# Neela08/cloud-security-pytorch-sagemaker-distributed-workshop

Hardware: AMD Instinct MI355X
Metric: images/sec (whole node) ResNet-50 DDP (higher is better)
Workload: dtype bf16; 1 GPU; model=resnet50, global_batch=256, per_gpu_batch=256, image_size=224, parallelism=dp1, optimizer=SGD(momentum=0.9, wd=1e-4), fp32 master weights, bf16 compute, backend=none, launcher=none, device=cuda, comm_forced_at_world1=False, buckets=5, grad_comm=fp32, wgrad_stream=True, hip_graph=False, gpu_max_hw_queues=8

## Files before the change

### csrc/kernels/gemm_conv.hip

```cpp
#include "common.h"
#include "epilogue.h"
#include <algorithm>
#include <array>
#include <climits>
#include <cstdio>
#include <vector>
#include <mutex>
#include <cstdlib>

constexpr int kNtBlocksPerCu = 4, kNt64BlocksPerCu = 4;
constexpr int kTnBlocksPerCu = 3, kTnConvBlocksPerCu = 3;
constexpr int kNtEpiEU = 4;

namespace {

struct ConvGeom {
  int H, W, Cs;
  int P, Q;
  int R, S, stride, pad;
  FastDiv fPQ, fQ, fS, fCpt;
  int Pc[4], Qc[4];
  FastDiv fPQc[4], fQc[4];
};

// ... 599 lines not shown
        float f[8];
        unpack8(v, f);
        if (a.epi == 5) {
          float c0[8];
          unpack8(cv[sl][u], c0);
#pragma unroll
          for (int q = 0; q < 8; ++q) f[q] += c0[q];
        }
        if constexpr (MASKC) {
          float xv[8];
          unpack8(xq[sl][u], xv);
#pragma unroll
          for (int q = 0; q < 8; ++q) {
            const float t = mthr[MASKC ? q : 0];
            const bool keep = ((mgt >> q) & 1u) ? xv[q] > t : xv[q] < t;
            f[q] = keep ? f[q] : 0.f;
          }
        } else if (a.bn_relu && a.mbits) {
#pragma unroll
          for (int q = 0; q < 8; ++q) f[q] = ((yq[sl][u].x >> q) & 1u) ? f[q] : 0.f;
        } else if (a.bn_relu) {
          float yv[8];
          unpack8(yq[sl][u], yv);
#pragma unroll
          for (int q = 0; q < 8; ++q) f[q] = yv[q] > 0.f ? f[q] : 0.f;
        }
        o = pack8(f);
        if (a.stats) {
          float xv[8];
          unpack8(xq[sl][u], xv);
#pragma unroll
          for (int q = 0; q < 8; ++q) { s1[q] += f[q]; s2[q] += f[q] * (xv[q] - mu[q]); }
        }
      } else {
        if (a.epi) o = epilogue_op_v(a.epi, v, a.aux + off, yq[sl][u]);
        if (a.stats) {
          float f[8];
          unpack8(v, f);
#pragma unroll
          for (int q = 0; q < 8; ++q) { s1[q] += f[q]; s2[q] += f[q] * f[q]; }
        }
      }
      *(uint4*)((bf16_t*)a.C + off) = o;
    }
  };
#pragma unroll
  for (int g = 0; g < NG; ++g) {
    load_grp(g, 0);
    proc_grp(g, 0);
  }
  if (a.stats) {
#pragma unroll
    for (int o = CPR; o < 64; o <<= 1) {
#pragma unroll
      for (int q = 0; q < 8; ++q) {
        s1[q] += __shfl_xor(s1[q], o, 64);
        s2[q] += __shfl_xor(s2[q], o, 64);
      }
    }
    if (lane < CPR) {
#pragma unroll
      for (int q = 0; q < 8; ++q) {
        Sred[(wid * 2 + 0) * BN + cc * 8 + q] = s1[q];
        Sred[(wid * 2 + 1) * BN + cc * 8 + q] = s2[q];
      }
    }
    __syncthreads();
    const int prow = cy * a.tiles_m + tm;
    for (int c = tid; c < 2 * BN; c += 256) {
      const int which = c / BN, col = c - which * BN;
      float t = 0.f;
#pragma unroll
      for (int w = 0; w < 4; ++w) t += Sred[(w * 2 + which) * BN + col];
      if (n0 + col < a.N) a.stats[((size_t)prow * 2 + which) * a.N + n0 + col] = t;
    }
  }
}

template <int UNITS>
__device__ __forceinline__ int tr_swz(int k) {
  return (4 * (k & 3) + 16 * ((k >> 3) & 1)) & (UNITS - 1);
}

template <int BM, int BN, int STAGES, int MODE = 1, bool CS = false, bool NOL = false, bool CSB = false>
__global__ __launch_bounds__(256, STAGES == 1 ? (MODE == 1 && !CS ? kTnConvBlocksPerCu : kTnBlocksPerCu) : 2)
void tn_kernel(TNArgs a) {
  static_assert(!CSB || (STAGES == 1 && !CS && !NOL), "folded BN backward: the plain one-stage variant");
  static_assert(!NOL || (MODE == 1 && STAGES == 1 && !CS), "normalize-on-load: conv weight gradients");
  constexpr int WM = BM / 2, WN = BN / 2;
  constexpr int MI = WM / 16, NJ = WN / 16;
  constexpr int AU = BM / 4, BU = BN / 4;
  constexpr int ACPR = BM / 8, BCPR = BN / 8;
  constexpr int A_CH = BK * ACPR / 256, B_CH = BK * BCPR / 256;
  constexpr int A_RSTEP = 256 / ACPR, B_RSTEP = 256 / BCPR;
  constexpr int A_RPI = 64 / ACPR, B_RPI = 64 / BCPR;
  __shared__ __attribute__((aligned(16))) uint2 smem[STAGES * BK * (AU + BU)];
  uint2* As = smem;
  uint2* Bs = smem + STAGES * BK * AU;

  const int nbn = (a.N + BN - 1) / BN;
  const int tiles = ((a.M + BM - 1) / BM) * nbn;
  const int nsplit = gridDim.x / tiles;
  const int w = xcd_remap(blockIdx.x, gridDim.x);
  const int split = w / tiles, tile = w - split * tiles;
  const int m0 = (tile / nbn) * BM, n0 = (tile % nbn) * BN;
  const int kbeg = split * a.k_per_split;
  const int kend = min(a.K, kbeg + a.k_per_split);
  if (kbeg >= kend) return;

  const int tid = threadIdx.x, lane = tid & 63, wid = tid >> 6;
  const int wm = wid >> 1, wn = wid & 1;
  const int a_cc = tid % ACPR, a_r = tid / ACPR;
  const int b_cc = tid % BCPR, b_r = tid / BCPR;
  const int a_lc = a_cc ^ (tr_swz<AU>(a_r) >> 1);
  const int b_lc = b_cc ^ (tr_swz<BU>(b_r) >> 1);

  int tap_r = 0, tap_s = 0, c0 = 0;
  if constexpr (MODE == 1) {
    const int ncol = n0 + b_lc * 8;
    const int tap = ncol / a.g.Cs;
    c0 = ncol - tap * a.g.Cs;
    tap_r = tap / a.g.S;
    tap_s = tap - tap_r * a.g.S;
  }
  const int H = a.g.H, W = a.g.W, P = a.g.P, Q = a.g.Q, Cs = a.g.Cs;
  const int st = a.g.stride, pad = a.g.pad;
  float nsc[NOL ? 8 : 1], nsh[NOL ? 8 : 1];
  if constexpr (NOL) {
    const bool live = n0 + b_lc * 8 < a.N;
#pragma unroll
    for (int q = 0; q < 8; ++q) {
      nsc[q] = live ? a.nol_scale[c0 + q] : 0.f;
      nsh[q] = live ? a.nol_shift[c0 + q] : 0.f;
    }
  }

  int b_img[B_CH], b_p[B_CH], b_q[B_CH];
#pragma unroll
  for (int i = 0; i < B_CH; ++i) {
    const uint32_t k = (uint32_t)min(kbeg + b_r + B_RSTEP * i, a.K - 1);
    if constexpr (MODE == 1) {
      const uint32_t img = fdiv(k, a.g.fPQ);
      const uint32_t rem = k - img * a.g.fPQ.d;
      const uint32_t p = fdiv(rem, a.g.fQ);
      b_img[i] = (int)img; b_p[i] = (int)p; b_q[i] = (int)(rem - p * a.g.fQ.d);
    } else {
      b_img[i] = b_p[i] = b_q[i] = 0;
    }
  }
  const int dq = BK % Q, dp = (BK / Q) % P, dimg = BK / (P * Q);

  const bool a_second = CSB && a.msplit && m0 >= a.msplit;
  const __amdgpu_buffer_rsrc_t rsA = __builtin_amdgcn_make_buffer_rsrc(
      (void*)(a_second ? a.A2 : a.A), (short)0, a_second ? a.a2_bytes : a.a_bytes, 0x00020000);
  const __amdgpu_buffer_rsrc_t rsB = __builtin_amdgcn_make_buffer_rsrc((void*)a.B, (short)0, a.b_bytes, 0x00020000);
  constexpr uint32_t OOB = 0xFFFFFFF0u;
  const int a_m = m0 + a_lc * 8;
  const int a_mo = a_second ? a_m - a.msplit : a_m;
  const int b_n = n0 + b_lc * 8;

  uint32_t b_okm = 0;
  auto issue_loads = [&](int k0, int buf) {
    b_okm = 0;
#pragma unroll
    for (int i = 0; i < A_CH; ++i) {
      const int k = k0 + a_r + A_RSTEP * i;
      const bool ok = k < kend && a_m < a.M;
      const uint32_t vo = ok ? (uint32_t)(k * (a_second ? a.lda2 : a.lda) + a_mo) * 2u : OOB;
      __builtin_amdgcn_raw_ptr_buffer_load_lds(
          rsA, LDS_PTR(void, &As[(buf * BK + A_RSTEP * i + wid * A_RPI) * AU]), 16, vo, 0, 0, 0);
    }
#pragma unroll
    for (int i = 0; i < B_CH; ++i) {
      const int k = k0 + b_r + B_RSTEP * i;
      uint32_t vo = OOB;
      if constexpr (MODE == 0) {
        if (k < kend && b_n < a.N) vo = (uint32_t)(k * a.ldb + b_n) * 2u;
      } else {
        const int ih = b_p[i] * st - pad + tap_r, iw = b_q[i] * st - pad + tap_s;
        if (k < kend && (unsigned)ih < (unsigned)H && (unsigned)iw < (unsigned)W)
          vo = (b_n < a.N) ? (uint32_t)((((b_img[i] * H + ih) * W + iw) * Cs) + c0) * 2u : OOB;
        b_okm |= (vo != OOB ? 1u : 0u) << i;
        int q = b_q[i] + dq, p = b_p[i] + dp, img = b_img[i] + dimg;
        if (q >= Q) { q -= Q; ++p; }
        if (p >= P) { p -= P; ++img; }
        b_q[i] = q; b_p[i] = p; b_img[i] = img;
      }
      __builtin_amdgcn_raw_ptr_buffer_load_lds(
          rsB, LDS_PTR(void, &Bs[(buf * BK + B_RSTEP * i + wid * B_RPI) * BU]), 16, vo, 0, 0, 0);
    }
  };

  f32x4 acc[MI][NJ];
#pragma unroll
  for (int i = 0; i < MI; ++i)
#pragma unroll
    for (int j = 0; j < NJ; ++j) acc[i][j] = f32x4{0.f, 0.f, 0.f, 0.f};

  const int g = lane >> 4, li = lane & 15, q4 = li >> 2, p4 = li & 3;
  const bool do_cs = CS && (tile % nbn) == 0 && wn == 0;
  f32x4 acc_cs[CS ? MI : 1];
#pragma unroll
  for (int i = 0; i < (CS ? MI : 1); ++i) acc_cs[i] = f32x4{0.f, 0.f, 0.f, 0.f};
  short ones_s __attribute__((ext_vector_type(8))) = {0x3F80, 0x3F80, 0x3F80, 0x3F80,
                                                      0x3F80, 0x3F80, 0x3F80, 0x3F80};
  const bf16x8 ones = __builtin_bit_cast(bf16x8, ones_s);
  const bool do_csb = CSB && tile / nbn == 0 && wm == 0;
  f32x4 acc_sb[CSB ? NJ : 1];
#pragma unroll
  for (int j = 0; j < (CSB ? NJ : 1); ++j) acc_sb[j] = f32x4{0.f, 0.f, 0.f, 0.f};
  auto compute = [&](int cur) {
#pragma unroll
    for (int kk = 0; kk < 2; ++kk) {
      bf16x8 af[MI], bfr[NJ];
      const int k1 = kk * 32 + 8 * g + q4;
      const int k2 = k1 + 4;
#pragma unroll
      for (int i = 0; i < MI; ++i) {
        const int u = (wm * WM + 16 * i) / 4 + p4;
        short4v lo = __builtin_amdgcn_ds_read_tr16_b64_v4i16(LDS_PTR(short4v, &As[(cur * BK + k1) * AU + (u ^ tr_swz<AU>(k1))]));
        short4v hi = __builtin_amdgcn_ds_read_tr16_b64_v4i16(LDS_PTR(short4v, &As[(cur * BK + k2) * AU + (u ^ tr_swz<AU>(k2))]));
        short v8 __attribute__((ext_vector_type(8))) = {lo[0], lo[1], lo[2], lo[3], hi[0], hi[1], hi[2], hi[3]};
        af[i] = __builtin_bit_cast(bf16x8, v8);
      }
#pragma unroll
      for (int j = 0; j < NJ; ++j) {
        const int u = (wn * WN + 16 * j) / 4 + p4;
        short4v lo = __builtin_amdgcn_ds_read_tr16_b64_v4i16(LDS_PTR(short4v, &Bs[(cur * BK + k1) * BU + (u ^ tr_swz<BU>(k1))]));
        short4v hi = __builtin_amdgcn_ds_read_tr16_b64_v4i16(LDS_PTR(short4v, &Bs[(cur * BK + k2) * BU + (u ^ tr_swz<BU>(k2))]));
        short v8 __attribute__((ext_vector_type(8))) = {lo[0], lo[1], lo[2], lo[3], hi[0], hi[1], hi[2], hi[3]};
        bfr[j] = __builtin_bit_cast(bf16x8, v8);
      }
#pragma unroll
      for (int i = 0; i < MI; ++i)
#pragma unroll
        for (int j = 0; j < NJ; ++j)
          acc[i][j] = __builtin_amdgcn_mfma_f32_16x16x32_bf16(af[i], bfr[j], acc[i][j], 0, 0, 0);
      if constexpr (CS) {
        if (do_cs)
#pragma unroll
        for (int i = 0; i < MI; ++i) acc_cs[i] = __builtin_amdgcn_mfma_f32_16x16x32_bf16(af[i], ones, acc_cs[i], 0, 0, 0);
      }
      if constexpr (CSB) {
        if (do_csb)
#pragma unroll
        for (int j = 0; j < NJ; ++j) acc_sb[j] = __builtin_amdgcn_mfma_f32_16x16x32_bf16(ones, bfr[j], acc_sb[j], 0, 0, 0);
      }
    }
  };

  const int nk = (kend - kbeg + BK - 1) / BK;
  if constexpr (STAGES == 1) {
    for (int kt = 0; kt < nk; ++kt) {
      issue_loads(kbeg + kt * BK, 0);
      asm volatile("s_waitcnt vmcnt(0)" ::: "memory");
      if constexpr (NOL) {
#pragma unroll
        for (int i = 0; i < B_CH; ++i) {
          if (!((b_okm >> i) & 1u)) continue;
          uint4* p = (uint4*)&Bs[(B_RSTEP * i + wid * B_RPI) * BU + 2 * lane];
          float f[8];
          unpack8(*p, f);
#pragma unroll
          for (int q = 0; q < 8; ++q) f[q] = fmaxf(fmaf(f[q], nsc[q], nsh[q]), 0.f);
          *p = pack8(f);
        }
      }
      __syncthreads();
      compute(0);
      __syncthreads();
    }
  } else {
    issue_loads(kbeg, 0);
    asm volatile("s_waitcnt vmcnt(0)" ::: "memory");
    __syncthreads();
    for (int kt = 0; kt < nk; ++kt) {
      const int cur = kt & 1;
      if (kt + 1 < nk) issue_loads(kbeg + (kt + 1) * BK, cur ^ 1);
      compute(cur);
      asm volatile("s_waitcnt vmcnt(0)" ::: "memory");
      __syncthreads();
    }
  }

  if constexpr (CS) if (do_cs && li == 0) {
#pragma unroll
    for (int i = 0; i < MI; ++i)
#pragma unroll
      for (int r = 0; r < 4; ++r) {
        const int m = m0 + wm * WM + 16 * i + 4 * g + r;
        if (m < a.M) atomicAdd(a.colsum + m, acc_cs[i][r]);
      }
  }

  if constexpr (CSB) if (do_csb && g == 0) {
#pragma unroll
    for (int j = 0; j < NJ; ++j) {
      const int n = n0 + wn * WN + 16 * j + li;
      if (n < a.N) a.bsum[(size_t)split * a.N + n] = acc_sb[j][0];
    }
  }

  const bool single = (nsplit == 1);
  if (!single && a.ws) {
    if (STAGES == 1 && a.cnt) {
      constexpr int FR = BM * BN / 4;
      constexpr int SC1 = 16;
      const __amdgpu_buffer_rsrc_t rsw = __builtin_amdgcn_make_buffer_rsrc(
          a.ws + (size_t)tile * nsplit * FR * 4, (short)0, nsplit * FR * 16, 0x00020000);
#pragma unroll
      for (int i = 0; i < MI; ++i)
#pragma unroll
        for (int j = 0; j < NJ; ++j)
          __builtin_amdgcn_raw_buffer_store_b128(
              acc[i][j], rsw, (uint32_t)((split * FR + ((i * NJ + j) * 4 + wid) * 64 + lane) * 16), 0, SC1);
      asm volatile("s_waitcnt vmcnt(0)" ::: "memory");
      __syncthreads();
      __shared__ int last_flag;
      if (tid == 0) last_flag = atomicAdd(a.cnt + tile, 1) == nsplit - 1;
      __syncthreads();
      if (!last_flag) return;
#pragma unroll
      for (int i = 0; i < MI; ++i)
#pragma unroll
        for (int j = 0; j < NJ; ++j) acc[i][j] = f32x4{0.f, 0.f, 0.f, 0.f};
      constexpr int IU = MI >= 2 ? MI / 2 : 1;
      for (int z = 0; z < nsplit; ++z) {
#pragma unroll
        for (int i0 = 0; i0 < MI; i0 += IU) {
          f32x4 r[IU][NJ];
#pragma unroll
          for (int i = 0; i < IU; ++i)
#pragma unroll
            for (int j = 0; j < NJ; ++j)
              r[i][j] = __builtin_amdgcn_raw_buffer_load_b128(
                  rsw, (uint32_t)((z * FR + (((i0 + i) * NJ + j) * 4 + wid) * 64 + lane) * 16), 0, SC1);
#pragma unroll
          for (int i = 0; i < IU; ++i)
#pragma unroll
            for (int j = 0; j < NJ; ++j) acc[i0 + i][j] += r[i][j];
        }
      }
      if (tid == 0) a.cnt[tile] = 0;
#pragma unroll
      for (int i = 0; i < MI; ++i) {
#pragma unroll
        for (int j = 0; j < NJ; ++j) {
          const int n = n0 + wn * WN + 16 * j + li;
          if (n >= a.N) continue;
          float c[4];
#pragma unroll
          for (int r = 0; r < 4; ++r) c[r] = a.C[(size_t)min(m0 + wm * WM + 16 * i + 4 * g + r, a.M - 1) * a.ldc + n];
#pragma unroll
          for (int r = 0; r < 4; ++r) {
            const int m = m0 + wm * WM + 16 * i + 4 * g + r;
            if (m < a.M) a.C[(size_t)m * a.ldc + n] = c[r] + acc[i][j][r];
          }
        }
      }
      return;
    }
    f32x4* slab = (f32x4*)a.ws + ((size_t)tile * nsplit + split) * (BM * BN / 4);
#pragma unroll
    for (int i = 0; i < MI; ++i)
#pragma unroll
      for (int j = 0; j < NJ; ++j) {
        f32x4* q = slab + ((i * NJ + j) * 4 + wid) * 64 + lane;
        *q = acc[i][j];
      }
  } else {
#pragma unroll
    for (int i = 0; i < MI; ++i) {
#pragma unroll
      for (int j = 0; j < NJ; ++j) {
        const int n = n0 + wn * WN + 16 * j + li;
        if (n >= a.N) continue;
#pragma unroll
        for (int r = 0; r < 4; ++r) {
          const int m = m0 + wm * WM + 16 * i + 4 * g + r;
          if (m >= a.M) continue;
          float* dst = a.C + (size_t)m * a.ldc + n;
          if (single) *dst += acc[i][j][r];
          else atomicAdd(dst, acc[i][j][r]);
        }
      }
    }
  }
}
// ... 393 lines not shown
                       int stats, int blocks, int splits) {
  if (g_trace_gemm < 0) {
    const char* e = std::getenv("MI355X_DP_TRACE_GEMM");
    g_trace_gemm = (e && e[0] == '1') ? 1 : 0;
  }
  if (!g_trace_gemm) return;
  static std::vector<std::array<int, 12>> seen;
  const std::array<int, 12> key{(int)(intptr_t)what, mode, M, N, K, Cs, R, stride, epi, stats, blocks, splits};
  for (auto& k : seen)
    if (k == key) return;
  seen.push_back(key);
  fprintf(stderr, "[gemm] %s mode=%d M=%d N=%d K=%d Cs=%d R=%d s=%d epi=%d stats=%d blocks=%d splits=%d\n", what,
          mode, M, N, K, Cs, R, stride, epi, stats, blocks, splits);
}

hipError_t dispatch_nt(NTArgs& a, hipStream_t st, const ConvRoute& r) {
  const ConvGeom& g = a.g;
  if (r.k == ConvKernel::NtHalo) {
    a.halo_rp = r.halo_rp;
    a.halo_pb = cdiv(g.P, r.halo_rp);
    a.fPB = make_fastdiv((uint32_t)a.halo_pb);
    a.fHW2 = make_fastdiv((uint32_t)(g.Q + 2));
    trace_gemm(r.bn == 64 ? "nt128x64-halo" : "nt128x128-halo", a.mode, a.M, a.N, a.K, g.Cs, g.R, g.stride, a.epi,
               a.stats != nullptr, (a.M / (g.P * g.Q)) * a.halo_pb, 1);
  } else {
    trace_gemm(r.bm == 64 ? "nt64x64" : (r.bn == 64 ? "nt128x64" : "nt128x128"), a.mode, a.M, a.N, a.K, g.Cs, g.R,
               g.stride, a.epi, a.stats != nullptr, cdiv(a.M, r.bm) * cdiv(a.N, r.bn), a.mode == 3 ? a.ncls : 1);
  }
  if (r.bm == 64) return launch_nt<64, 64>(a, st);
  return r.bn == 64 ? launch_nt<128, 64>(a, st) : launch_nt<128, 128>(a, st);
}
hipError_t dispatch_nt(NTArgs& a, hipStream_t st) { return dispatch_nt(a, st, nt_route(a.M, a.N)); }

struct SplitkWs { float* p = nullptr; size_t n = 0; };
static SplitkWs g_splitk_ws[16][3];
static hipStream_t g_wgrad_stream[16];
static hipStream_t g_aux_stream[16];
static std::mutex g_splitk_mu;
static float* splitk_workspace(size_t floats, hipStream_t st) {
  int dev = 0;
  hipGetDevice(&dev);
  std::lock_guard<std::mutex> lk(g_splitk_mu);
  const int slot = st == nullptr ? 0 : st == g_wgrad_stream[dev & 15] ? 1 : st == g_aux_stream[dev & 15] ? 2 : 0;
  SplitkWs& w = g_splitk_ws[dev & 15][slot];
  if (w.n < floats) {
    if (mi_stream_capturing(st)) {
      mi_ws_capture_warn("split-K slab");
      return nullptr;
    }
    const size_t n = std::max(floats, (size_t)16 << 20);
    float* p = nullptr;
    if (hipMalloc(&p, n * sizeof(float)) != hipSuccess) return nullptr;
    mi_ws_retire(w.p);
    w.p = p;
    w.n = n;
  }
  return w.p;
}
static int* g_splitk_cnt[16][3];
static int* splitk_counters(hipStream_t st) {
  int dev = 0;
  hipGetDevice(&dev);
  std::lock_guard<std::mutex> lk(g_splitk_mu);
  const int slot = st == nullptr ? 0 : st == g_wgrad_stream[dev & 15] ? 1 : st == g_aux_stream[dev & 15] ? 2 : 0;
  int*& p = g_splitk_cnt[dev & 15][slot];
  if (!p) {
    if (hipMalloc(&p, sizeof(int) * SPLITK_COUNTERS) != hipSuccess) { p = nullptr; return nullptr; }
    if (hipMemset(p, 0, sizeof(int) * SPLITK_COUNTERS) != hipSuccess) return nullptr;
  }
  return p;
}
extern "C" float* mi_partials_workspace(size_t floats, hipStream_t st) { return splitk_workspace(floats, st); }
MI_API int mi_splitk_ws_reserve(size_t floats, hipStream_t st) { return splitk_workspace(floats, st) ? 0 : 1; }
static int g_tn_slabs = -1;
static bool tn_slabs_on() {
  if (g_tn_slabs < 0) {
    const char* e = std::getenv("MI355X_DP_TN_SLABS");
    g_tn_slabs = (e && e[0] == '0') ? 0 : 1;
  }
  return g_tn_slabs != 0;
}

static int g_tn_stages = -1;
static int tn_stages() {
  if (g_tn_stages < 0) {
    const char* e = std::getenv("MI355X_DP_TN_STAGES");
    g_tn_stages = (e && e[0] == '2') ? 2 : 1;
  }
  return g_tn_stages;
}

template <int BM, int BN>
hipError_t launch_tn(TNArgs& a, hipStream_t st, int target_blocks) {
  int tiles = cdiv(a.M, BM) * cdiv(a.N, BN);
  int ksteps = cdiv(a.K, BK);
  int splits = std::max(1, std::min(ksteps, target_blocks / std::max(tiles, 1)));
  int steps_per = cdiv(ksteps, splits);
  a.k_per_split = steps_per * BK;
  splits = cdiv(a.K, a.k_per_split);
  trace_gemm(BM == 128 ? (BN == 128 ? "tn128x128" : "tn128x64") : (BN == 128 ? "tn64x128" : "tn64x64"), a.mode,
             a.M, a.N, a.K, a.g.Cs, a.g.R, a.g.stride, 0, 0, tiles, splits);
  if (a.a_bytes <= 0 || a.b_bytes <= 0) return hipErrorInvalidValue;
  a.ws = nullptr;
  a.cnt = nullptr;
  if (splits > 1 && tn_slabs_on())
    a.ws = splitk_workspace((size_t)tiles * splits * BM * BN, st);
  const int st_n = glds_on() ? tn_stages() : 2;
  if (a.ws && splits < 8 && tiles <= SPLITK_COUNTERS && st_n == 1 && tn_split_fused() && !a.nol_scale)
    a.cnt = splitk_counters(st);
  if (a.nol_scale) {
    if (a.mode != 1 || st_n != 1 || a.cnt) return hipErrorNotSupported;
    hipLaunchKernelGGL((tn_kernel<BM, BN, 1, 1, false, true>), dim3(tiles * splits), dim3(256), 0, st, a);
  } else if (a.mode == 1 && a.bsum) {
    hipLaunchKernelGGL((tn_kernel<BM, BN, 1, 1, false, false, true>), dim3(tiles * splits), dim3(256), 0, st, a);
  } else if (a.mode == 1) {
    if (st_n == 1) hipLaunchKernelGGL((tn_kernel<BM, BN, 1, 1, false>), dim3(tiles * splits), dim3(256), 0, st, a);
    else hipLaunchKernelGGL((tn_kernel<BM, BN, 2, 1, false>), dim3(tiles * splits), dim3(256), 0, st, a);
  } else if (a.colsum) {
    if (st_n == 1) hipLaunchKernelGGL((tn_kernel<BM, BN, 1, 0, true>), dim3(tiles * splits), dim3(256), 0, st, a);
    else hipLaunchKernelGGL((tn_kernel<BM, BN, 2, 0, true>), dim3(tiles * splits), dim3(256), 0, st, a);
  } else {
    if (st_n == 1) hipLaunchKernelGGL((tn_kernel<BM, BN, 1, 0, false>), dim3(tiles * splits), dim3(256), 0, st, a);
    else hipLaunchKernelGGL((tn_kernel<BM, BN, 2, 0, false>), dim3(tiles * splits), dim3(256), 0, st, a);
  }
  if (a.ws && !a.cnt) {
    int log2g = 0;
    while (log2g < 6 && (splits >> (log2g + 3)) > 0) ++log2g;
    const int pb = 256 >> log2g;
    hipLaunchKernelGGL((tn_splitk_reduce_kernel<BM, BN>), dim3(cdiv(BM * BN / 4, pb), tiles), dim3(256), 0, st,
                       (const f32x4*)a.ws, a.C, a.M, a.N, a.ldc, cdiv(a.N, BN), splits, log2g);
  }
  return hipGetLastError();
}

static int g_tn_blocks = -1, g_tn_blocks_side = -1;
static int tn_target_blocks(hipStream_t st) {
  if (g_tn_blocks < 0) {
    const char* e = std::getenv("MI355X_DP_TN_BLOCKS");
    g_tn_blocks = e ? std::max(64, std::atoi(e)) : 768;
    const char* es = std::getenv("MI355X_DP_TN_BLOCKS_SIDE");
    g_tn_blocks_side = es ? std::max(64, std::atoi(es)) : (e ? g_tn_blocks : 384);
  }
  int dev = 0;
  hipGetDevice(&dev);
  return (st != nullptr && st == g_wgrad_stream[dev & 15]) ? g_tn_blocks_side : g_tn_blocks;
}

hipError_t dispatch_tn(TNArgs& a, hipStream_t st) {
  const int target = tn_target_blocks(st);
  bool n64 = a.N <= 64;
  bool m64 = a.M <= 64;
  if (m64 && n64) return launch_tn<64, 64>(a, st, target);
  if (m64) return launch_tn<64, 128>(a, st, target);
  if (n64) return launch_tn<128, 64>(a, st, target);
  return launch_tn<128, 128>(a, st, target);
}

}

MI_API int mi_register_wgrad_stream(hipStream_t st) {
  int dev = 0;
  hipGetDevice(&dev);
  std::lock_guard<std::mutex> lk(g_splitk_mu);
  g_wgrad_stream[dev & 15] = st;
  return 0;
}

MI_API int mi_register_aux_stream(hipStream_t st) {
  int dev = 0;
  hipGetDevice(&dev);
  std::lock_guard<std::mutex> lk(g_splitk_mu);
  g_aux_stream[dev & 15] = st;
  return 0;
}

MI_API int mi_create_cu_masked_stream(int ncu, int spread, hipStream_t* out) {
  int dev = 0, total = 0;
  hipGetDevice(&dev);
  if (hipDeviceGetAttribute(&total, hipDeviceAttributeMultiprocessorCount, dev) != hipSuccess || total <= 0)
    return (int)hipErrorInvalidValue;
  ncu = std::max(1, std::min(ncu, total));
  std::vector<uint32_t> mask((total + 31) / 32, 0u);
  for (int k = 0; k < ncu; ++k) {
    const int cu = spread ? (int)((int64_t)k * total / ncu) : k;
    mask[cu / 32] |= 1u << (cu % 32);
  }
  return (int)hipExtStreamCreateWithCUMask(out, (uint32_t)mask.size(), mask.data());
}

MI_API int mi_set_tn_slabs(int on) {
  g_tn_slabs = on ? 1 : 0;
  return 0;
}

MI_API int mi_set_glds(int on) {
  g_nt_glds = on ? 1 : 0;
  return 0;
}

MI_API int mi_set_tn_split_fused(int on) {
  g_tn_split_fused = on ? 1 : 0;
  return 0;
}
MI_API int mi_set_nt_split_fused(int on) {
  g_nt_split_fused = on ? 1 : 0;
  return 0;
}

MI_API int mi_set_nt_split_blocks(int blocks) {
  g_nt_split_blocks = std::max(0, blocks);
  return 0;
}

MI_API int mi_set_nt_stages(int stages) {
  g_nt_stages = stages == 2 ? 2 : 1;
  return 0;
}

MI_API void mi_set_panel_first(int on) { sw().panel_first = on ? 1 : 0; }
MI_API void mi_set_conv256_min_tiles(int t) { sw().conv256_min_tiles = t; }
MI_API void mi_set_conv256_min_k(int k) { sw().conv256_min_k = k; }
MI_API void mi_set_ds256(int on) { sw().ds256 = on ? 1 : 0; }
MI_API void mi_set_wgrad256(int min_tiles) { sw().wgrad256 = std::max(0, min_tiles); }
MI_API void mi_set_gemm256(int on) { sw().gemm256 = on ? 1 : 0; }

extern "C" int mi_gemm256_conv(int mode, const void* A, const void* B, void* C, float* stats, int epi, void* aux,
                               const void* aux2, const float* mean, int bn_relu, int Nb, int H, int W, int Cs,
                               int P, int Q, int R, int S, int stride, int pad, int N, int aux_even,
                               const void* mbits, hipStream_t st);
extern "C" int mi_gemm256_nt_scat2(const void* A, const void* B, void* C, int M, int N, int K, int Q, int W,
                                   hipStream_t st);
extern "C" int mi_panel_conv(const void* x, const void* w, void* y, float* stats, int Nb, int H, int W, int C, int K,
                             int R, int stride, int pad, int P, int Q, hipStream_t st);
extern "C" int mi_panel_dgrad(const void* dy, const void* wt, void* dx, int Nb, int H, int W, int C, int K, int R,
                              int epi, const void* aux, const void* aux2, const float* mean, int bn_relu, float* stats,
                              int aux_even, const void* mbits, const void* acc_src, hipStream_t st);
extern "C" int mi_stem_conv_fwd(const void* x, const void* w, void* y, float* stats, int Nb, int H, int W, int P,
                                int Q, int pad, hipStream_t st);
extern "C" int mi_stem_wgrad(const void* x, const void* dy, float* dw, int Nb, int H, int W, int P, int Q, int pad,
                             hipStream_t st);

MI_API int mi_conv_stat_rows_g(int Nb, int H, int W, int C, int K, int R, int S, int stride, int pad, int P, int Q) {
  return route_fwd(Nb, H, W, C, K, R, S, stride, pad, P, Q).stat_rows;
}
MI_API int mi_conv_stat_rows(int M, int N, int Cs, int RS) {
  return route_fwd(M, 1, 1, Cs, N, 1, RS, 1, 0, 1, 1).stat_rows;
}
MI_API int mi_dgrad_stat_rows_g(int Nb, int H, int W, int C, int K, int R, int S, int stride, int pad, int P, int Q) {
  return route_dgrad(Nb, H, W, C, K, R, S, stride, pad, P, Q, 4, 0).stat_rows;
}
MI_API int mi_dgrad_stat_rows(int Nb, int H, int W, int C, int P, int Q, int stride, int K, int RS) {
  int R = 1;
  while ((R + 1) * (R + 1) <= RS) ++R;
  return mi_dgrad_stat_rows_g(Nb, H, W, C, K, R, R, stride, R / 2, P, Q);
}

MI_API int mi_conv2d_fwd(const void* x, const void* w, void* y, const float* bias, float* stats,
                         int Nb, int H, int W, int C, int K, int R, int S,
                         int stride, int pad, int P, int Q, int out_f32, hipStream_t st) {
  if ((C % 64 != 0 && C != 8) || K % 8 != 0) return (int)hipErrorInvalidValue;
  const ConvRoute r = route_fwd(Nb, H, W, C, K, R, S, stride, pad, P, Q, out_f32 || bias);
  switch (r.k) {
    case ConvKernel::Stem: return mi_stem_conv_fwd(x, w, y, stats, Nb, H, W, P, Q, pad, st);
    case ConvKernel::G256:
      return mi_gemm256_conv(1, x, w, y, stats, 0, nullptr, nullptr, nullptr, 0, Nb, H, W, C, P, Q, R, S, stride, pad,
                             K, 0, nullptr, st);
    case ConvKernel::Panel: return mi_panel_conv(x, w, y, stats, Nb, H, W, C, K, R, stride, pad, P, Q, st);
    default: break;
  }
  NTArgs a{};
  a.A = (const bf16_t*)x; a.B = (const bf16_t*)w; a.C = y; a.bias = bias; a.stats = stats;
  a.M = Nb * P * Q; a.N = K; a.K = R * S * C;
  a.lda = 0; a.ldb = a.K; a.ldc = K; a.mode = (C == 8) ? 4 : 1; a.out_f32 = out_f32; a.accumulate = 0;
  a.a_bytes = rsrc_bytes((int64_t)Nb * H * W * C);
  a.b_bytes = rsrc_bytes((int64_t)K * a.K);
  a.g = make_geom(H, W, C, P, Q, S, stride, pad, R);
  return (int)dispatch_nt(a, st, r);
}

MI_API int mi_conv2d_dgrad_ex4(const void* dy, const void* wt, void* dx, int Nb, int H, int W, int C, int K, int R,
                               int S, int stride, int pad, int P, int Q, int epi, const void* aux, const void* aux2,
                               const float* mean, int bn_relu, float* stats, int flags, const float* mask_scale,
                               const float* mask_shift, const void* mbits, hipStream_t st) {
  const bool mask_c = mask_scale != nullptr;
// ... 306 lines not shown
```

### mi355x_dp/ops/kernels.py

```python
from ._lib import signature, c_void_p as P, c_int as I, c_int64 as L, c_float as F
import ctypes

U32 = ctypes.c_uint32

signature("mi_conv2d_fwd", P, P, P, P, P, I, I, I, I, I, I, I, I, I, I, I, I, P)
signature("mi_set_glds", I)
signature("mi_set_nt_stages", I)
signature("mi_set_nt_split_blocks", I)
signature("mi_set_nt_split_fused", I)
signature("mi_set_tn_split_fused", I)
signature("mi_conv2d_dgrad", P, P, P, I, I, I, I, I, I, I, I, I, I, I, P)
signature("mi_conv2d_wgrad", P, P, P, I, I, I, I, I, I, I, I, I, I, I, P)
signature("mi_conv_nol_ok", I, I, I, I, I, I, I, I, I, I, I)
signature("mi_conv2d_fwd_nol", P, P, P, P, P, P, I, I, I, I, I, I, I, I, I, I, I, P)
signature("mi_conv2d_wgrad_nol", P, P, P, P, P, I, I, I, I, I, I, I, I, I, I, I, P)
signature("mi_conv2d_dgrad_ex3", P, P, P, I, I, I, I, I, I, I, I, I, I, I, I, P, P, P, I, P, I, P, P, P)
signature("mi_conv2d_dgrad_ex4", P, P, P, I, I, I, I, I, I, I, I, I, I, I, I, P, P, P, I, P, I, P, P, P, P)
signature("mi_set_gemm256", I)
signature("mi_set_conv256_min_tiles", I)
signature("mi_set_conv256_min_k", I)
signature("mi_set_panel_first", I)
signature("mi_set_wgrad256", I)
signature("mi_set_ds256", I)
signature("mi_conv_stat_rows_g", I, I, I, I, I, I, I, I, I, I, I)
signature("mi_conv_stat_rows", I, I, I, I)
signature("mi_dgrad_stat_rows_g", I, I, I, I, I, I, I, I, I, I, I)
signature("mi_dgrad_stat_rows", I, I, I, I, I, I, I, I, I)
signature("mi_conv_fbb_route", I, I, I)
signature("mi_conv_fbb_rows", I, I, I)
signature("mi_conv2d_dgrad_ex", P, P, P, I, I, I, I, I, I, I, I, I, I, I, I, P, P, P, I, P, P)
signature("mi_conv2d_dgrad_ex2", P, P, P, I, I, I, I, I, I, I, I, I, I, I, I, P, P, P, I, P, I, P)
signature("mi_conv_wtrans", P, P, I, I, I, P)
signature("mi_stem_wpack", P, P, I, I, I, I, L, L, L, L, P)
signature("mi_stem_wgrad_to", P, P, P, I, L, L, L, L, I, I, I, I, I, I, I, I, I, I, P)
signature("mi_conv_wtrans_multi", P, P, P, I, I, P)
signature("mi_gemm_nt", P, P, P, P, P, I, I, I, I, I, I, I, I, P)
signature("mi_gemm_tn", P, P, P, I, I, I, I, I, I, P)
signature("mi_gemm_tn_bias", P, P, P, P, I, I, I, I, I, I, P)
signature("mi_register_wgrad_stream", P)
signature("mi_register_aux_stream", P)
signature("mi_create_cu_masked_stream", I, I, P)
signature("mi_splitk_ws_reserve", ctypes.c_size_t, P)

signature("mi_bn_partial_rows", I, I)
signature("mi_bn_slab_extra_rows")
signature("mi_bn_set_small_elems", L)
signature("mi_bn_init_counters")
signature("mi_bn_fwd_train", P, P, P, I, I, F, F, P, P, P, P, P, P, P, P, P, P, I, I, P)
signature("mi_bn_apply_dual", P, P, P, I, I, P, P, P, P, I, P)
signature("mi_bn_apply_bits", P, P, P, P, I, I, P, P, P, P, P)
signature("mi_bn_fwd_eval", P, P, P, I, I, F, P, P, P, P, P, P, I, P)
signature("mi_bn_bwd_train", P, P, P, P, P, I, I, P, P, P, P, P, P, P, I, P)
signature("mi_bn_bwd_eval", P, P, P, P, P, I, I, I, P)
signature("mi_bnpool_partial_rows", I, I)
signature("mi_bnpool_fwd", P, P, P, P, P, I, I, I, I, I, I, I, I, I, P)
signature("mi_bnpool_bwd", P, P, P, P, I, I, I, I, I, I, I, I, I, P, P, P, P, P, P, P, P, P, P)

signature("mi_maxpool_fwd", P, P, P, I, I, I, I, I, I, I, I, I, P)
signature("mi_maxpool_bwd", P, P, P, I, I, I, I, I, I, I, I, I, P)
signature("mi_gap_fwd", P, P, I, I, I, P)
signature("mi_gap_bwd", P, P, I, I, I, P)
signature("mi_ce_fwd", P, P, P, P, I, I, I, P)
signature("mi_ce_bwd", P, P, P, P, P, I, I, I, I, I, P)
signature("mi_sgd_flat", P, P, P, P, L, F, F, F, F, I, I, F, P)
signature("mi_cast_bf16", P, P, L, P)
signature("mi_augment", P, P, I, I, I, I, I, I, I, U32, P, P, P)
signature("mi_im2col", P, P, I, I, I, I, I, I, I, I, I, I, I, P)
signature("mi_add_bf16", P, P, P, L, P)
signature("mi_checksum", P, L, P, P)
signature("mi_flags_alloc", I, P)
signature("mi_flag_bump", P, P)
signature("mi_flag_gate", P, U32, P, I, P)
signature("mi_host_word_alloc", P, P)
signature("mi_capture_enter", restype=None)
signature("mi_capture_exit", restype=None)
signature("mi_capture_depth")

D = ctypes.c_double
signature("mi_grad_sqnorm_blocks", L)
signature("mi_grad_sqnorm_partial", P, L, P, P)
signature("mi_grad_sqnorm_final", P, I, P, P)
signature("mi_adamw_prep", P, P, D, D, D, D, D, I, P)
signature("mi_adamw_flat", P, P, P, P, P, L, P, P, L, D, D, D, P)
signature("mi_seg_sqnorm_units", P, P, L, P, P, P)
signature("mi_seg_sqnorm_reduce", P, L, I, P, I, P, P)
signature("mi_lars_trust", P, P, P, P, I, D, D, D, D, P)
signature("mi_lamb_trust", P, P, P, I, P)
signature("mi_lars_flat", P, P, P, P, L, P, P, P, P, L, D, D, D, P)
signature("mi_lamb_prep", P, P, D, D, D, D, I, P)
signature("mi_lamb_moments", P, P, P, P, L, P, P, P, L, P, P, D, D, D, D, P)
signature("mi_lamb_apply", P, P, P, P, L, P, P, P, P, L, D, D, D, D, P)

signature("mi_gemm_nt_epi", P, P, P, P, P, I, I, I, I, I, I, I, P)
# ... 66 lines not shown
```

Before: 13860 images/s.

## Replace two-stage TN weight-gradient loop with a multi-slot LDS ring using counted waits

Rewrites the STAGES==2 path of the TN (weight-gradient) GEMM/conv kernel as a 3–4 slot ring of 32-row K chunks. It uses a counted vmcnt wait and a raw barrier, so several global-to-LDS loads stay in flight while the current slot is computed, replacing the full drain-and-sync on every iteration. Conv-mode weight gradients now default to this ring path, and it also serves the folded-BN variant and the fused split-K counter path. The aim is to hide memory latency in wgrad, at the cost of more LDS per block, which could reduce occupancy. The hand-written waits and barriers also carry correctness risk.

```diff
diff --git a/csrc/kernels/gemm_conv.hip b/csrc/kernels/gemm_conv.hip
--- a/csrc/kernels/gemm_conv.hip
+++ b/csrc/kernels/gemm_conv.hip
@@ -705,21 +705,48 @@
   return (4 * (k & 3) + 16 * ((k >> 3) & 1)) & (UNITS - 1);
 }
 
+constexpr int kTnRingRows = 32;
+template <int BM, int BN>
+constexpr int tn_ring_slots() {
+  return BM + BN >= 256 ? 3 : 4;
+}
+
+template <int BM, int BN, int STAGES, int MODE, bool CS>
+constexpr int tn_blocks_per_cu() {
+  constexpr int one = MODE == 1 && !CS ? kTnConvBlocksPerCu : kTnBlocksPerCu;
+  static_assert(STAGES == 1 || 160 * 1024 / (tn_ring_slots<BM, BN>() * kTnRingRows * (BM + BN) * 2 + 64) >= one,
+                "the ring's LDS must leave the launch bound's blocks resident in a CU's 160 KB");
+  return one;
+}
+
+template <int N>
+__device__ __forceinline__ void tn_vmwait() {
+  static_assert(N > 0 && N <= 63, "counted wait: vmcnt holds 6 bits, and 0 would drain the ring");
+  asm volatile("s_waitcnt vmcnt(%0)" ::"n"(N) : "memory");
+}
+
+typedef uint32_t tn_u32x2 __attribute__((ext_vector_type(2)));
+
 template <int BM, int BN, int STAGES, int MODE = 1, bool CS = false, bool NOL = false, bool CSB = false>
-__global__ __launch_bounds__(256, STAGES == 1 ? (MODE == 1 && !CS ? kTnConvBlocksPerCu : kTnBlocksPerCu) : 2)
+__global__ __launch_bounds__(256, (tn_blocks_per_cu<BM, BN, STAGES, MODE, CS>()))
 void tn_kernel(TNArgs a) {
-  static_assert(!CSB || (STAGES == 1 && !CS && !NOL), "folded BN backward: the plain one-stage variant");
+  static_assert(STAGES == 1 || STAGES == 2, "one-stage loop or the slot ring");
+  static_assert(!CSB || (!CS && !NOL), "folded BN backward: the plain variants");
   static_assert(!NOL || (MODE == 1 && STAGES == 1 && !CS), "normalize-on-load: conv weight gradients");
+  constexpr bool RING = STAGES == 2;
+  constexpr int KS = RING ? kTnRingRows : BK;
+  constexpr int NBUF = RING ? tn_ring_slots<BM, BN>() : 1;
   constexpr int WM = BM / 2, WN = BN / 2;
   constexpr int MI = WM / 16, NJ = WN / 16;
   constexpr int AU = BM / 4, BU = BN / 4;
   constexpr int ACPR = BM / 8, BCPR = BN / 8;
-  constexpr int A_CH = BK * ACPR / 256, B_CH = BK * BCPR / 256;
+  constexpr int A_CH = KS * ACPR / 256, B_CH = KS * BCPR / 256;
   constexpr int A_RSTEP = 256 / ACPR, B_RSTEP = 256 / BCPR;
   constexpr int A_RPI = 64 / ACPR, B_RPI = 64 / BCPR;
-  __shared__ __attribute__((aligned(16))) uint2 smem[STAGES * BK * (AU + BU)];
+  static_assert(A_CH >= 1 && B_CH >= 1 && A_CH * A_RSTEP == KS && B_CH * B_RSTEP == KS, "whole passes per issue");
+  __shared__ __attribute__((aligned(16))) uint2 smem[NBUF * KS * (AU + BU)];
   uint2* As = smem;
-  uint2* Bs = smem + STAGES * BK * AU;
+  uint2* Bs = smem + NBUF * KS * AU;
 
   const int nbn = (a.N + BN - 1) / BN;
   const int tiles = ((a.M + BM - 1) / BM) * nbn;
@@ -771,7 +798,7 @@
       b_img[i] = b_p[i] = b_q[i] = 0;
     }
   }
-  const int dq = BK % Q, dp = (BK / Q) % P, dimg = BK / (P * Q);
+  const int dq = KS % Q, dp = (KS / Q) % P, dimg = KS / (P * Q);
 
   const bool a_second = CSB && a.msplit && m0 >= a.msplit;
   const __amdgpu_buffer_rsrc_t rsA = __builtin_amdgcn_make_buffer_rsrc(
@@ -791,7 +818,7 @@
       const bool ok = k < kend && a_m < a.M;
       const uint32_t vo = ok ? (uint32_t)(k * (a_second ? a.lda2 : a.lda) + a_mo) * 2u : OOB;
       __builtin_amdgcn_raw_ptr_buffer_load_lds(
-          rsA, LDS_PTR(void, &As[(buf * BK + A_RSTEP * i + wid * A_RPI) * AU]), 16, vo, 0, 0, 0);
+          rsA, LDS_PTR(void, &As[(buf * KS + A_RSTEP * i + wid * A_RPI) * AU]), 16, vo, 0, 0, 0);
     }
 #pragma unroll
     for (int i = 0; i < B_CH; ++i) {
@@ -810,7 +837,7 @@
         b_q[i] = q; b_p[i] = p; b_img[i] = img;
       }
       __builtin_amdgcn_raw_ptr_buffer_load_lds(
-          rsB, LDS_PTR(void, &Bs[(buf * BK + B_RSTEP * i + wid * B_RPI) * BU]), 16, vo, 0, 0, 0);
+          rsB, LDS_PTR(void, &Bs[(buf * KS + B_RSTEP * i + wid * B_RPI) * BU]), 16, vo, 0, 0, 0);
     }
   };
 
@@ -832,6 +859,23 @@
   f32x4 acc_sb[CSB ? NJ : 1];
 #pragma unroll
   for (int j = 0; j < (CSB ? NJ : 1); ++j) acc_sb[j] = f32x4{0.f, 0.f, 0.f, 0.f};
+  auto mma_chunk = [&](const bf16x8 (&af)[MI], const bf16x8 (&bfr)[NJ]) {
+#pragma unroll
+    for (int i = 0; i < MI; ++i)
+#pragma unroll
+      for (int j = 0; j < NJ; ++j)
+        acc[i][j] = __builtin_amdgcn_mfma_f32_16x16x32_bf16(af[i], bfr[j], acc[i][j], 0, 0, 0);
+    if constexpr (CS) {
+      if (do_cs)
+#pragma unroll
+      for (int i = 0; i < MI; ++i) acc_cs[i] = __builtin_amdgcn_mfma_f32_16x16x32_bf16(af[i], ones, acc_cs[i], 0, 0, 0);
+    }
+    if constexpr (CSB) {
+      if (do_csb)
+#pragma unroll
+      for (int j = 0; j < NJ; ++j) acc_sb[j] = __builtin_amdgcn_mfma_f32_16x16x32_bf16(ones, bfr[j], acc_sb[j], 0, 0, 0);
+    }
+  };
   auto compute = [&](int cur) {
 #pragma unroll
     for (int kk = 0; kk < 2; ++kk) {
@@ -854,22 +898,47 @@
         short v8 __attribute__((ext_vector_type(8))) = {lo[0], lo[1], lo[2], lo[3], hi[0], hi[1], hi[2], hi[3]};
         bfr[j] = __builtin_bit_cast(bf16x8, v8);
       }
-#pragma unroll
-      for (int i = 0; i < MI; ++i)
-#pragma unroll
-        for (int j = 0; j < NJ; ++j)
-          acc[i][j] = __builtin_amdgcn_mfma_f32_16x16x32_bf16(af[i], bfr[j], acc[i][j], 0, 0, 0);
-      if constexpr (CS) {
-        if (do_cs)
-#pragma unroll
-        for (int i = 0; i < MI; ++i) acc_cs[i] = __builtin_amdgcn_mfma_f32_16x16x32_bf16(af[i], ones, acc_cs[i], 0, 0, 0);
-      }
-      if constexpr (CSB) {
-        if (do_csb)
-#pragma unroll
-        for (int j = 0; j < NJ; ++j) acc_sb[j] = __builtin_amdgcn_mfma_f32_16x16x32_bf16(ones, bfr[j], acc_sb[j], 0, 0, 0);
-      }
-    }
+      mma_chunk(af, bfr);
+    }
+  };
+
+  uint32_t fa[RING ? MI : 1], fb[RING ? NJ : 1];
+  if constexpr (RING) {
+    const int k1 = 8 * g + q4;
+#pragma unroll
+    for (int i = 0; i < MI; ++i)
+      fa[i] = (uint32_t)(uintptr_t)LDS_PTR(void, &As[k1 * AU + (((wm * WM + 16 * i) / 4 + p4) ^ tr_swz<AU>(k1))]);
+#pragma unroll
+    for (int j = 0; j < NJ; ++j)
+      fb[j] = (uint32_t)(uintptr_t)LDS_PTR(void, &Bs[k1 * BU + (((wn * WN + 16 * j) / 4 + p4) ^ tr_swz<BU>(k1))]);
+  }
+  auto compute_slot = [&](int cur) {
+    tn_u32x2 alo[MI], ahi[MI], blo[NJ], bhi[NJ];
+#pragma unroll
+    for (int i = 0; i < MI; ++i)
+      asm volatile("ds_read_b64_tr_b16 %0, %2\n\tds_read_b64_tr_b16 %1, %2 offset:%3"
+                   : "=&v"(alo[i]), "=&v"(ahi[i])
+                   : "v"(fa[RING ? i : 0] + (uint32_t)(cur * KS * AU * 8)), "n"(4 * AU * 8)
+                   : "memory");
+#pragma unroll
+    for (int j = 0; j < NJ; ++j)
+      asm volatile("ds_read_b64_tr_b16 %0, %2\n\tds_read_b64_tr_b16 %1, %2 offset:%3"
+                   : "=&v"(blo[j]), "=&v"(bhi[j])
+                   : "v"(fb[RING ? j : 0] + (uint32_t)(cur * KS * BU * 8)), "n"(4 * BU * 8)
+                   : "memory");
+    asm volatile("s_waitcnt lgkmcnt(0)" ::: "memory");
+    bf16x8 af[MI], bfr[NJ];
+#pragma unroll
+    for (int i = 0; i < MI; ++i) {
+      asm volatile("" : "+v"(alo[i]), "+v"(ahi[i]));
+      af[i] = __builtin_bit_cast(bf16x8, __builtin_shufflevector(alo[i], ahi[i], 0, 1, 2, 3));
+    }
+#pragma unroll
+    for (int j = 0; j < NJ; ++j) {
+      asm volatile("" : "+v"(blo[j]), "+v"(bhi[j]));
+      bfr[j] = __builtin_bit_cast(bf16x8, __builtin_shufflevector(blo[j], bhi[j], 0, 1, 2, 3));
+    }
+    mma_chunk(af, bfr);
   };
 
   const int nk = (kend - kbeg + BK - 1) / BK;
@@ -894,16 +963,22 @@
       __syncthreads();
     }
   } else {
-    issue_loads(kbeg, 0);
+    constexpr int S = NBUF;
+    static_assert(S >= 3, "at least one slot in flight behind the wait");
+    constexpr int LPS = A_CH + B_CH;
+    const int ns = 2 * nk;
+#pragma unroll
+    for (int s = 0; s < S - 1; ++s) issue_loads(kbeg + s * KS, s);
+    int cur = 0, prev = S - 1;
+    for (int t = 0; t < ns; ++t) {
+      tn_vmwait<(S - 2) * LPS>();
+      asm volatile("s_barrier" ::: "memory");
+      issue_loads(kbeg + (t + S - 1) * KS, prev);
+      compute_slot(cur);
+      prev = cur;
+      cur = cur + 1 == S ? 0 : cur + 1;
+    }
     asm volatile("s_waitcnt vmcnt(0)" ::: "memory");
-    __syncthreads();
-    for (int kt = 0; kt < nk; ++kt) {
-      const int cur = kt & 1;
-      if (kt + 1 < nk) issue_loads(kbeg + (kt + 1) * BK, cur ^ 1);
-      compute(cur);
-      asm volatile("s_waitcnt vmcnt(0)" ::: "memory");
-      __syncthreads();
-    }
   }
 
   if constexpr (CS) if (do_cs && li == 0) {
@@ -926,7 +1001,7 @@
 
   const bool single = (nsplit == 1);
   if (!single && a.ws) {
-    if (STAGES == 1 && a.cnt) {
+    if (a.cnt) {
       constexpr int FR = BM * BN / 4;
       constexpr int SC1 = 16;
       const __amdgpu_buffer_rsrc_t rsw = __builtin_amdgcn_make_buffer_rsrc(
@@ -1486,12 +1561,12 @@
 }
 
 static int g_tn_stages = -1;
-static int tn_stages() {
+static int tn_stages(int mode) {
   if (g_tn_stages < 0) {
     const char* e = std::getenv("MI355X_DP_TN_STAGES");
-    g_tn_stages = (e && e[0] == '2') ? 2 : 1;
-  }
-  return g_tn_stages;
+    g_tn_stages = (e && e[0] == '2') ? 2 : (e && e[0] == '1') ? 1 : 0;
+  }
+  return g_tn_stages ? g_tn_stages : (mode == 1 ? 2 : 1);
 }
 
 template <int BM, int BN>
@@ -1509,14 +1584,15 @@
   a.cnt = nullptr;
   if (splits > 1 && tn_slabs_on())
     a.ws = splitk_workspace((size_t)tiles * splits * BM * BN, st);
-  const int st_n = glds_on() ? tn_stages() : 2;
-  if (a.ws && splits < 8 && tiles <= SPLITK_COUNTERS && st_n == 1 && tn_split_fused() && !a.nol_scale)
+  const int st_n = glds_on() ? tn_stages(a.mode) : 1;
+  if (a.ws && splits < 8 && tiles <= SPLITK_COUNTERS && glds_on() && tn_split_fused() && !a.nol_scale)
     a.cnt = splitk_counters(st);
   if (a.nol_scale) {
-    if (a.mode != 1 || st_n != 1 || a.cnt) return hipErrorNotSupported;
+    if (a.mode != 1 || !glds_on() || a.cnt) return hipErrorNotSupported;
     hipLaunchKernelGGL((tn_kernel<BM, BN, 1, 1, false, true>), dim3(tiles * splits), dim3(256), 0, st, a);
   } else if (a.mode == 1 && a.bsum) {
-    hipLaunchKernelGGL((tn_kernel<BM, BN, 1, 1, false, false, true>), dim3(tiles * splits), dim3(256), 0, st, a);
+    if (st_n == 1) hipLaunchKernelGGL((tn_kernel<BM, BN, 1, 1, false, false, true>), dim3(tiles * splits), dim3(256), 0, st, a);
+    else hipLaunchKernelGGL((tn_kernel<BM, BN, 2, 1, false, false, true>), dim3(tiles * splits), dim3(256), 0, st, a);
   } else if (a.mode == 1) {
     if (st_n == 1) hipLaunchKernelGGL((tn_kernel<BM, BN, 1, 1, false>), dim3(tiles * splits), dim3(256), 0, st, a);
     else hipLaunchKernelGGL((tn_kernel<BM, BN, 2, 1, false>), dim3(tiles * splits), dim3(256), 0, st, a);
@@ -1604,6 +1680,10 @@
 
 MI_API int mi_set_tn_split_fused(int on) {
   g_tn_split_fused = on ? 1 : 0;
+  return 0;
+}
+MI_API int mi_set_tn_stages(int stages) {
+  g_tn_stages = (stages == 1 || stages == 2) ? stages : -1;
   return 0;
 }
 MI_API int mi_set_nt_split_fused(int on) {
diff --git a/mi355x_dp/ops/kernels.py b/mi355x_dp/ops/kernels.py
--- a/mi355x_dp/ops/kernels.py
+++ b/mi355x_dp/ops/kernels.py
@@ -9,6 +9,7 @@
 signature("mi_set_nt_split_blocks", I)
 signature("mi_set_nt_split_fused", I)
 signature("mi_set_tn_split_fused", I)
+signature("mi_set_tn_stages", I)
 signature("mi_conv2d_dgrad", P, P, P, I, I, I, I, I, I, I, I, I, I, I, P)
 signature("mi_conv2d_wgrad", P, P, P, I, I, I, I, I, I, I, I, I, I, I, P)
 signature("mi_conv_nol_ok", I, I, I, I, I, I, I, I, I, I, I)
```

New measurement: 14030 images/s, median of 6. 1.01x the previous value.
